# Lillthorin/YoloLite-Official-Repo

Hardware: AMD Instinct MI355X
Metric: images/sec (higher is better)
Workload: dtype f32

## Files before the change

yololite-official-repo_amd/_lib.py:

```python
from __future__ import annotations

import ctypes as C
import os
import sys
import warnings


def _default_hw_queues():
    if "GPU_MAX_HW_QUEUES" in os.environ or os.environ.get("YOLOLITE_NO_ENV_DEFAULTS"):
        return
    os.environ["GPU_MAX_HW_QUEUES"] = "8"
    t = sys.modules.get("torch")
    try:
        late = t is not None and t.cuda.is_initialized()
    except Exception:
        late = False
    if late:
        warnings.warn("yololite_amd: the HIP runtime was initialised before this package was imported, so "
                      "GPU_MAX_HW_QUEUES=8 cannot be applied; export it in the environment (multi-stream overlap "
                      "of the executor degrades by ~25 % next to RCCL streams otherwise)", RuntimeWarning)


_default_hw_queues()

_HERE = os.path.dirname(os.path.abspath(__file__))
LIB_PATH = os.environ.get("YOLOLITE_HIP_LIB") or os.path.join(_HERE, "libyololite_hip.so")

YL_ABI_VERSION = 5
YL_MAX_LEVELS = 8
YL_OK = 0
ACT = {"none": 0, "relu": 1, "relu6": 2, "silu": 3, "gelu": 4, "relu_lab": 5}
OP_STEM, OP_CONV, OP_DW, OP_STEMBLOCK, OP_SE = 0, 1, 2, 3, 4
OP_POOL, OP_COPY, OP_LN, OP_GRN, OP_NHWC4 = 5, 6, 7, 8, 9
POST_MAIN, POST_FALLBACK, POST_EVAL = 0, 1, 2
CENTER = {"v8": 0, "simple": 1}
WH = {"softplus": 0, "v8": 1, "exp": 2}
NMS_TORCHVISION, NMS_GREEDY = 0, 1

DEV_DW_TILE_OFF, DEV_PWS_OFF, DEV_S2C_OFF, DEV_DWC_ALL, DEV_DWT_OFF = 1, 2, 4, 8, 16
DEV_DWT_NOSPLIT = 1 << 10
DEV_WINO_V1 = 1 << 11
DEV_DWL_OFF = 1 << 14
DEV_DWL_ALL = 1 << 15
DEV_DPW_OFF = 1 << 16
DEV_K3W_OFF = 1 << 17
DEV_POISON = 1 << 18
DEV_WINO_SHAPE_SHIFT = 12

_fp = C.POINTER(C.c_float)
_ip = C.POINTER(C.c_int32)


class yl_layer(C.Structure):
    _fields_ = [(n, C.c_int32) for n in (
        "op", "in_slot", "out_slot", "res_slot", "up_slot", "head_level", "cin", "cout",
        "k", "stride", "pad_t", "pad_l", "act", "in_shift", "dw_k", "dw_stride", "dw_pad_t", "dw_pad_l", "dw_act")] + [
        ("w", _fp), ("b", _fp), ("dw_w", _fp), ("dw_b", _fp),
        ("c2", C.c_int32), ("act2", C.c_int32), ("c3", C.c_int32), ("act3", C.c_int32),
        ("w2", _fp), ("b2", _fp), ("w3", _fp), ("b3", _fp), ("scale_slot", C.c_int32), ("reserved0", C.c_int32),
        ("lab_scale", C.c_float), ("lab_bias", C.c_float), ("eps", C.c_float), ("out_ch_off", C.c_int32)]


class yl_model_desc(C.Structure):
    _fields_ = [("abi_version", C.c_int32), ("img_size", C.c_int32), ("in_channels", C.c_int32),
                ("num_classes", C.c_int32), ("num_masks", C.c_int32), ("proto_slot", C.c_int32),
                ("num_levels", C.c_int32),
                ("level_size", C.c_int32 * YL_MAX_LEVELS), ("level_anchors", C.c_int32 * YL_MAX_LEVELS),
                ("num_slots", C.c_int32), ("slot_h", _ip), ("slot_w", _ip), ("slot_c", _ip),
                ("num_layers", C.c_int32), ("layers", C.POINTER(yl_layer))]


class yl_post_cfg(C.Structure):
    _fields_ = [("mode", C.c_int32), ("conf_thr", C.c_float), ("iou_thr", C.c_float),
                ("per_class_cap", C.c_int32), ("topk", C.c_int32), ("max_out", C.c_int32),
                ("center_mode", C.c_int32), ("wh_mode", C.c_int32), ("backmap_dev", C.c_void_p),
                ("fallback_nms", C.c_int32)]


_vp = C.c_void_p
# ... 79 lines not shown
```

yololite-official-repo_amd/csrc/yl_api.hip:

```cpp
#include "yl_internal.h"

#include <dlfcn.h>
#include <limits.h>
#include <math.h>
#include <stdio.h>
#include <stddef.h>
#include <string.h>

#include <algorithm>
#include <memory>
#include <chrono>
#include <string>
#include <vector>

#define YL_DW_LDS_MAX (32 * 1024)

namespace {

struct DevLayer {
  yl_layer d;
  float* wp = nullptr;
  float* bias = nullptr;
  float* dw_w = nullptr;
  float* dw_b = nullptr;
// ... 40 lines not shown
  bool plan_reuse = false;
  int opt_reuse = 1;
  int opt_time_split = 0;
  hipEvent_t ev_t[3] = {nullptr, nullptr, nullptr};
  bool timing_valid = false;
  int opt_pre_norm = 0;
  float* level_buf[YL_MAX_LEVELS] = {nullptr};
  float4* ws_boxes = nullptr;
  float* ws_scores = nullptr;
  int* ws_cls = nullptr;
  int* ws_clsws = nullptr;
  int* ws_kept_list = nullptr;
  int* ws_done = nullptr;
  unsigned long long* ws_gkeys = nullptr;
  int gP = 0;
  float* ws_tmp_dets = nullptr;
  int* ws_tmp_idx = nullptr;
  int post_cap_batch = 0;
  int* ws_nms_clsws = nullptr;
  unsigned long long* ws_nms_gkeys = nullptr;
  int nms_gP = 0;
  int opt_graph = 0, opt_tile_m = 0, opt_streams = 2;
  int opt_nms_groups = 0;
  int opt_hybrid = 0;
  int small_lo = 0, small_hi = 0;
  int tiny_lo = 0, tiny_hi = 0;
  int opt_batch_levels = 1;
  int opt_winograd = 1;
  int wino_max_hw = 0;
  int opt_fuse_decode = 1;
  int opt_fuse_head = 1;
  int opt_split_k = 0;
  int opt_dev = 0;
  int opt_bf16 = 0;
  hipStream_t work[4] = {nullptr, nullptr, nullptr, nullptr};
  hipEvent_t ev_fork = nullptr, ev_join[4] = {nullptr, nullptr, nullptr, nullptr};
  int opt_lanes = 0;
  std::vector<unsigned char> lane;
  hipStream_t side[4] = {nullptr, nullptr, nullptr, nullptr};
  hipEvent_t ev_la[4] = {nullptr, nullptr, nullptr, nullptr}, ev_lb[4] = {nullptr, nullptr, nullptr, nullptr};
  struct GraphEntry {
    std::vector<hipGraphExec_t> execs;
    int n = 0;
    std::vector<unsigned char> key;
    unsigned long long stamp = 0;
  };
  std::vector<GraphEntry> graphs;
  unsigned long long graph_clock = 0;
  std::shared_ptr<int> weights_owner;
  std::string err;
};

namespace {

bool g_inited[64] = {false};

yl_status fail(yl_ctx* c, yl_status s, const std::string& msg) {
  if (c) c->err = msg;
  return s;
}

#define HIPCHK(ctx, expr)                                                                        \
  do {                                                                                           \
    hipError_t _e = (expr);                                                                      \
    if (_e != hipSuccess) {                                                                      \
      char _b[512];                                                                              \
// ... 116 lines not shown
    hipFree(c->arena[i]); c->arena[i] = nullptr; c->arena_capi[i] = 0;
    hipFree(c->se_scratch[i]); c->se_scratch[i] = nullptr;
  }
  for (auto& s : c->slots) { hipFree(s.pin); s.pin = nullptr; }
  for (int l = 0; l < YL_MAX_LEVELS; ++l) { hipFree(c->level_buf[l]); c->level_buf[l] = nullptr; }
  c->cap_batch = 0; c->plan_n = 0; c->arena_n = 0; c->arena_cap = 0; c->act_batch = 0;
}

int pow2ceil(int v) { int p = 64; while (p < v) p <<= 1; return p; }

size_t layer_group_end(const yl_ctx* c, size_t i, size_t lend) {
  auto same_shape = [&](size_t x, size_t y) {
    const yl_layer& a = c->layers[x].d; const yl_layer& e = c->layers[y].d;
    return a.op == YL_OP_CONV && e.op == YL_OP_CONV && a.cin == e.cin && a.cout == e.cout && a.k == e.k &&
           a.stride == e.stride && a.pad_t == e.pad_t && a.pad_l == e.pad_l && a.act == e.act &&
           !YL_ACT_POSTPASS(a.act) && a.in_shift == e.in_shift && a.dw_k == e.dw_k && a.dw_stride == e.dw_stride && a.dw_pad_t == e.dw_pad_t &&
           a.dw_pad_l == e.dw_pad_l && a.dw_act == e.dw_act && a.c2 == 0 && e.c2 == 0 && a.scale_slot < 0 && e.scale_slot < 0 && a.res_slot < 0 &&
           e.res_slot < 0 && a.up_slot < 0 && e.up_slot < 0 && (a.head_level >= 0) == (e.head_level >= 0) &&
           (a.cout + 15) / 16 <= 8;
  };
  size_t gend = i + 1;
  if (c->layers[i].d.op != YL_OP_CONV) return gend;
  while (gend < lend && gend - i < 4 && same_shape(i, gend)) {
    bool dep = false;
    for (size_t q = i; q < gend; ++q)
      if (c->layers[q].d.head_level < 0 && c->layers[q].d.out_slot == c->layers[gend].d.in_slot) dep = true;
    if (dep) break;
    ++gend;
  }
  return gend;
}

bool pair_fusable(const yl_ctx* c, size_t i, size_t lend, bool ignore_options);

void plan_slots(yl_ctx* c, bool reuse) {
  const size_t NL = c->layers.size(), NS = c->slots.size();
  std::vector<int> grp(NL, 0);
  int g = 0;
  for (size_t i = 0; i < NL; ++g) {
    size_t e = layer_group_end(c, i, NL);
    if (pair_fusable(c, e - 1, NL, true)) e = e + 1;
    for (size_t q = i; q < e; ++q) grp[q] = g;
    i = e;
  }
  const int INF = 1 << 30;
  std::vector<int> def(NS, INF), last(NS, -1);
  for (size_t i = 0; i < NL; ++i) {
    const yl_layer& d = c->layers[i].d;
    if (d.head_level < 0 && d.out_slot >= 0 && grp[i] < def[d.out_slot]) def[d.out_slot] = grp[i];
    const int ins[4] = {(d.op == YL_OP_STEM || d.op == YL_OP_STEMBLOCK || d.op == YL_OP_NHWC4) ? -1 : d.in_slot, d.res_slot, d.up_slot, d.scale_slot};
    for (int k = 0; k < 4; ++k)
      if (ins[k] >= 0 && grp[i] > last[ins[k]]) last[ins[k]] = grp[i];
  }
  for (size_t s = 0; s < NS; ++s) {
    Slot& t = c->slots[s];
    t.pinned = (int)s == c->proto_slot;
    bool f32 = c->opt_bf16 != 3 || t.pinned;
    for (size_t i = 0; i < NL && !f32; ++i) f32 = c->layers[i].d.op == YL_OP_SE && c->layers[i].d.out_slot == (int)s;
    t.sz = (size_t)t.h * t.w * t.c * (f32 ? sizeof(float) : sizeof(_Float16));
    if (last[s] < def[s]) last[s] = def[s] == INF ? -1 : def[s];
  }
  struct Iv { size_t off, sz; int last; };
  std::vector<Iv> live;
  size_t peak = 0;
  std::vector<size_t> order;
  for (size_t s = 0; s < NS; ++s) if (!c->slots[s].pinned && def[s] != INF) order.push_back(s);
  std::stable_sort(order.begin(), order.end(), [&](size_t a, size_t b) { return def[a] < def[b]; });
  size_t bump = 0;
  for (size_t s : order) {
    Slot& t = c->slots[s];
    const size_t need = (t.sz + 255) & ~(size_t)255;
    if (!reuse) { t.off = bump; bump += need; peak = bump; continue; }
    live.erase(std::remove_if(live.begin(), live.end(), [&](const Iv& v) { return v.last < def[s]; }), live.end());
    std::sort(live.begin(), live.end(), [](const Iv& a, const Iv& b) { return a.off < b.off; });
// ... 214 lines not shown
      return false;
    if (T.in_h != T.out_h || T.in_w != T.out_w || !yl_dpp_supported(t.cin, t.cout, o.cout, T.out_h, T.out_w)) return false;
    for (size_t r = 0; r < c->layers.size(); ++r) {
      if (r == gend + q) continue;
      const yl_layer& e = c->layers[r].d;
      const bool reads_in = e.op != YL_OP_STEM && e.op != YL_OP_STEMBLOCK && e.in_slot == t.out_slot;
      if (reads_in || e.res_slot == t.out_slot || e.up_slot == t.out_slot) return false;
    }
  }
  return true;
}

bool pair_fusable(const yl_ctx* c, size_t i, size_t lend, bool ignore_options) {
  if ((!ignore_options && (!c->opt_fuse_head || c->opt_bf16)) || i + 1 >= lend) return false;
  const DevLayer& T = c->layers[i];
  const yl_layer& t = T.d; const yl_layer& o = c->layers[i + 1].d;
  if (t.op != YL_OP_CONV || t.k != 1 || t.dw_k != 3 || t.dw_stride != 1 || t.c2 > 0 || t.c3 > 0 || t.head_level >= 0 ||
      t.res_slot >= 0 || t.up_slot >= 0 || t.in_shift || YL_SMOOTH(t.act) || YL_SMOOTH(t.dw_act) || t.out_slot < 0)
    return false;
  if (o.op != YL_OP_CONV || o.head_level >= 0 || o.k != 1 || o.dw_k > 0 || o.c2 > 0 || o.c3 > 0 || o.in_slot != t.out_slot ||
      o.cin != t.cout || YL_SMOOTH(o.act) || o.up_slot >= 0 || o.in_shift || o.res_slot == t.out_slot ||
      o.scale_slot >= 0 || t.scale_slot >= 0)
    return false;
  if (T.in_h != T.out_h || T.in_w != T.out_w || !yl_dpq_supported(t.cin, t.cout, o.cout, T.out_h, T.out_w)) return false;
  for (size_t r = 0; r < c->layers.size(); ++r) {
    if (r == i + 1) continue;
    const yl_layer& e = c->layers[r].d;
    const bool reads_in = e.op != YL_OP_STEM && e.op != YL_OP_STEMBLOCK && e.in_slot == t.out_slot;
    if (reads_in || e.res_slot == t.out_slot || e.up_slot == t.out_slot) return false;
  }
  return true;
}

hipError_t conv_multi(const yl_ctx* c, const YlConvP* ps, int n, hipStream_t st) {
  switch (c->opt_bf16) {
    case 1: return yl_launch_conv_multi_bf16(ps, n, c->opt_tile_m, st);
    case 2: return yl_launch_conv_multi_f16(ps, n, c->opt_tile_m, st);
    case 3: return yl_launch_conv_multi_f16s(ps, n, c->opt_tile_m, st);
    default: return yl_launch_conv_multi(ps, n, c->opt_tile_m, st);
  }
}

yl_status run_layers(yl_ctx* c, const float* x, int b0, int B, float* const* level_out, hipStream_t st,
                     hipEvent_t* evs , int chunk = 0,
                     const yl_post_cfg* fuse = nullptr ,
                     int lo = 0, int hi = -1 ) {
  if (evs) HIPCHK(c, hipEventRecord(evs[0], st));
  const bool lanes = !evs && c->opt_lanes && !c->lane.empty() && chunk >= 0 && chunk < 4;
  hipStream_t sd = nullptr;
  if (lanes) {
    if (!c->side[chunk]) HIPCHK(c, hipStreamCreateWithFlags(&c->side[chunk], hipStreamNonBlocking));
    if (!c->ev_la[chunk]) HIPCHK(c, hipEventCreateWithFlags(&c->ev_la[chunk], hipEventDisableTiming));
    if (!c->ev_lb[chunk]) HIPCHK(c, hipEventCreateWithFlags(&c->ev_lb[chunk], hipEventDisableTiming));
    sd = c->side[chunk];
  }
  std::vector<unsigned char> prod(c->slots.size(), 0);
  bool side_used = false;
  int pooled_slot = -1, pooled_P = 0;
  auto params = [&](size_t i, YlConvP& p) {
    layer_params(c, c->layers[i], b0, B, x, level_out, p);
    const yl_layer& d = c->layers[i].d;
    if (fuse && d.head_level >= 0) {
      const int l = d.head_level, S = c->level_S[l];
      const size_t o = (size_t)b0 * c->N;
      p.dec_boxes = c->ws_boxes + o; p.dec_scores = c->ws_scores + o; p.dec_cls = c->ws_cls + o;
      p.dec_N = c->N; p.dec_off = c->level_off[l] + c->layers[i].head_anchor * S * S; p.dec_C = c->C;
// ... 31 lines not shown
      const hipError_t e = yl_launch_conv_dpp(ps, (int)n, st);
      if (e == hipSuccess) { i = gend + n; continue; }
      if (e != hipErrorNotSupported) {
        char b[256];
        snprintf(b, sizeof(b), "layers %zu..%zu head launch failed: %s", i, gend + n - 1, hipGetErrorString(e));
        return fail(c, YL_ERR_HIP, b);
      }
    }
    if (!evs && !lanes && gend == i + 1 && d.op == YL_OP_CONV && d.dw_k == 3 && d.dw_stride == 1 && d.k == 1 && d.c2 == 0 &&
        d.c3 == 0 && c->opt_fuse_head && !c->opt_bf16 && d.head_level < 0 && d.res_slot < 0 && d.up_slot < 0 && !d.in_shift &&
        d.cout > 96 && !pair_fusable(c, i, lend, false) && c->layers[i].in_h == c->layers[i].out_h &&
        yl_dpq_supported(d.cin, d.cout, 0, c->layers[i].out_h, c->layers[i].out_w)) {
      YlConvP pt;
      params(i, pt);
      pt.w3p = nullptr;
      const hipError_t e = yl_launch_conv_dpq(pt, st);
      if (e == hipSuccess) { ++i; continue; }
      if (e != hipErrorNotSupported) {
        char b[256];
        snprintf(b, sizeof(b), "layer %zu launch failed: %s", i, hipGetErrorString(e));
        return fail(c, YL_ERR_HIP, b);
      }
    }
    if (!evs && !lanes && gend == i + 1 && d.op == YL_OP_CONV && d.dw_k == 3 && pair_fusable(c, i, lend, false)) {
      YlConvP pt, po;
      params(i, pt);
      params(i + 1, po);
      pt.w3p = po.wp; pt.b3 = po.bias; pt.C3 = po.N; pt.act3 = po.act; pt.res = po.res; pt.out = po.out;
      const hipError_t e = yl_launch_conv_dpq(pt, st);
      if (e == hipSuccess) { i += 2; continue; }
      if (e != hipErrorNotSupported) {
        char b[256];
        snprintf(b, sizeof(b), "layers %zu..%zu fused launch failed: %s", i, i + 1, hipGetErrorString(e));
        return fail(c, YL_ERR_HIP, b);
      }
    }
    if (fuse && !evs && !lanes && d.op == YL_OP_CONV && d.head_level >= 0 && c->layers[i].wp_det && c->opt_fuse_head) {
      bool all = true;
      for (size_t q = i; q < gend; ++q) all = all && c->layers[q].wp_det != nullptr;
      if (all) {
        YlConvP pd[4];
        const int nd = 5 + c->C;
        for (size_t q = i; q < gend; ++q) {
          YlConvP o;
          params(q, o);
          YlConvP& a = pd[q - i];
          a = o; a.wp = c->layers[q].wp_det; a.bias = c->layers[q].b_det; a.N = nd; a.NTtot = cdiv(nd, 16); a.dec_raw = 0;
          a.w3p = c->layers[q].wp_mc; a.b3 = c->layers[q].b_mc; a.C3 = c->NM;
          a.out = o.out + nd; a.ldo = c->E;
        }
        const int n = (int)(gend - i);
        const hipError_t e = conv_multi(c, pd, n, st);
        if (e != hipSuccess) {
          char b[256];
          snprintf(b, sizeof(b), "layers %zu..%zu split head launch failed: %s", i, gend - 1, hipGetErrorString(e));
          return fail(c, YL_ERR_HIP, b);
        }
        i = gend;
        continue;
      }
    }
    if (gend - i > 1) {
      YlConvP ps[4];
      for (size_t q = i; q < gend; ++q) params(q, ps[q - i]);
      const hipError_t e = conv_multi(c, ps, (int)(gend - i), st);
      if (e != hipSuccess) {
// ... 863 lines not shown
    const int nv = value ? 3 : (c->opt_bf16 == 3 ? 0 : c->opt_bf16);
    if ((nv == 3) != (c->opt_bf16 == 3)) free_act(c);
    c->opt_bf16 = nv; drop_graph(c); return YL_OK;
  }
  if (!strcmp(name, "nms_groups")) { c->opt_nms_groups = value < 0 ? 0 : (value > YL_NMS_GROUPS ? YL_NMS_GROUPS : value); drop_graph(c); return YL_OK; }
  if (!strcmp(name, "time_split")) {
    c->opt_time_split = value ? 1 : 0;
    for (int i = 0; i < 3 && value; ++i)
      if (!c->ev_t[i]) HIPCHK(c, hipEventCreate(&c->ev_t[i]));
    c->timing_valid = false;
    return YL_OK;
  }
  if (!strcmp(name, "pre_norm")) { c->opt_pre_norm = value ? 1 : 0; return YL_OK; }
  if (!strcmp(name, "reuse_slots")) { c->opt_reuse = value ? 1 : 0; drop_graph(c); return YL_OK; }
  if (!strcmp(name, "hybrid")) { c->opt_hybrid = value < 0 ? 0 : (value > 2 ? 2 : value); drop_graph(c); return YL_OK; }
  if (!strcmp(name, "batch_levels")) { c->opt_batch_levels = value ? 1 : 0; drop_graph(c); return YL_OK; }
  if (!strcmp(name, "fuse_decode")) { c->opt_fuse_decode = value ? 1 : 0; drop_graph(c); return YL_OK; }
  if (!strcmp(name, "fuse_head")) { c->opt_fuse_head = value ? 1 : 0; drop_graph(c); return YL_OK; }
  if (!strcmp(name, "winograd")) { c->opt_winograd = value < 0 ? 0 : (value > 2 ? 2 : value); drop_graph(c); return YL_OK; }
  if (!strcmp(name, "lanes")) { c->opt_lanes = value ? 1 : 0; drop_graph(c); return YL_OK; }
  if (!strcmp(name, "tile_m")) { c->opt_tile_m = value; drop_graph(c); return YL_OK; }
  if (!strcmp(name, "streams")) { c->opt_streams = value < 1 ? 1 : (value > 4 ? 4 : value); drop_graph(c); return YL_OK; }
  if (!strcmp(name, "split_k")) { c->opt_split_k = value ? 1 : 0; drop_graph(c); return YL_OK; }
  if (!strcmp(name, "dev_select")) { c->opt_dev = value & (int)YL_DEV_MASK; drop_graph(c); return YL_OK; }
  return fail(c, YL_ERR_INVALID, std::string("unknown option ") + name);
}

yl_status yl_get_option(const yl_ctx* c, const char* name, int32_t* value) {
  if (!c || !name || !value) return YL_ERR_INVALID;
  const struct { const char* n; int v; } tab[] = {
      {"graph", c->opt_graph}, {"mfma_bf16", c->opt_bf16 == 1}, {"mfma_f16", c->opt_bf16 == 2}, {"store_f16", c->opt_bf16 == 3}, {"nms_groups", c->opt_nms_groups}, {"time_split", c->opt_time_split},
      {"pre_norm", c->opt_pre_norm}, {"reuse_slots", c->opt_reuse}, {"hybrid", c->opt_hybrid}, {"batch_levels", c->opt_batch_levels},
      {"fuse_decode", c->opt_fuse_decode}, {"fuse_head", c->opt_fuse_head}, {"winograd", c->opt_winograd}, {"lanes", c->opt_lanes},
      {"tile_m", c->opt_tile_m}, {"streams", c->opt_streams}, {"dev_select", c->opt_dev}, {"split_k", c->opt_split_k}};
  for (const auto& t : tab)
    if (!strcmp(name, t.n)) { *value = t.v; return YL_OK; }
  return YL_ERR_INVALID;
}

int32_t yl_query_fused_block(int32_t c_in, int32_t c_mid, int32_t c_out, int32_t dw_k, int32_t dw_stride, int32_t out_h,
                             int32_t out_w) {
  if (c_in < 1 || c_mid < 1 || c_out < 1 || out_h < 1 || out_w < 1) return 0;
  if (yl_ir_supported(c_in, c_mid, c_out, dw_k, dw_stride, out_h, out_w)) return 1;
  if (dw_stride == 1 && !(out_h & 3) && !(out_w & 3) && yl_uib_supported(c_in, c_mid, c_out, dw_k)) return 2;
  return 0;
}

int32_t yl_query_dw_prologue(int32_t c_in, int32_t c_out, int32_t dw_k, int32_t dw_stride, int32_t out_h, int32_t out_w) {
  if (c_in < 1 || c_out < 1 || dw_k < 1 || dw_stride < 1 || out_h < 1 || out_w < 1) return 0;
  if (yl_dws_supported(c_in, c_out, dw_k, dw_stride, out_h, out_w)) return 2;
  if ((size_t)(dw_k * dw_k + 1) * c_in * sizeof(float) <= YL_DW_LDS_MAX) return 1;
  return 0;
}

static yl_status forward_impl(yl_ctx* c, const float* x, int B, float* const* level_out, hipStream_t st,
                              float* layer_ms, const yl_post_cfg* cfg, float* dets, int* counts, int* keep_idx = nullptr) {
  if (!c) return YL_ERR_INVALID;
  if (c->layers.empty()) return fail(c, YL_ERR_STATE, "context was created without layers");
  if (!x || B < 1) return fail(c, YL_ERR_INVALID, "bad input");
  HIPCHK(c, hipSetDevice(c->device));
  yl_status s = ensure_act(c, B, layer_ms ? 1 : chunks_for(c, B));
  if (s != YL_OK) return s;
  if (cfg && (s = ensure_post(c, B)) != YL_OK) return s;
  if ((s = poison_act(c, st)) != YL_OK) return s;
  Job j;
  j.x = x; j.B = B; j.cfg = cfg; j.dets = dets; j.counts = counts; j.keep_idx = keep_idx;
  for (int l = 0; l < c->L; ++l) j.outs[l] = (level_out && level_out[l]) ? level_out[l] : c->level_buf[l];
// ... 206 lines not shown
```

yololite-official-repo_amd/csrc/yl_convc.hip:

```cpp
#include "yl_lp.h"
#if defined(YL_BF16) && YL_BF16
#define yl_conv_dwc_kernel YL_LP_NAME(yl_conv_dwc_kernel)
#define yl_launch_conv_dwc YL_LP_NAME(yl_launch_conv_dwc)
#define yl_convc_init YL_LP_NAME(yl_convc_init)
#define yl_conv_pwt_kernel YL_LP_NAME(yl_conv_pwt_kernel)
#define yl_launch_conv_pwt YL_LP_NAME(yl_launch_conv_pwt)
#define yl_launch_conv_pwt_multi YL_LP_NAME(yl_launch_conv_pwt_multi)
#define yl_conv_dwt_kernel YL_LP_NAME(yl_conv_dwt_kernel)
#define yl_launch_conv_dwt YL_LP_NAME(yl_launch_conv_dwt)
#define yl_conv_dwk_kernel YL_LP_NAME(yl_conv_dwk_kernel)
#define yl_conv_dwl_kernel YL_LP_NAME(yl_conv_dwl_kernel)
#define yl_launch_conv_dwk YL_LP_NAME(yl_launch_conv_dwk)
#define yl_conv_dws_kernel YL_LP_NAME(yl_conv_dws_kernel)
#define yl_launch_conv_dws YL_LP_NAME(yl_launch_conv_dws)
#define yl_conv_wino_kernel YL_LP_NAME(yl_conv_wino_kernel)
#define yl_launch_conv_wino YL_LP_NAME(yl_launch_conv_wino)
#define yl_conv_kxk_kernel YL_LP_NAME(yl_conv_kxk_kernel)
#define yl_launch_conv_kxk YL_LP_NAME(yl_launch_conv_kxk)
#define yl_conv_pws_kernel YL_LP_NAME(yl_conv_pws_kernel)
#define yl_launch_conv_pws YL_LP_NAME(yl_launch_conv_pws)
#define yl_ir_kernel YL_LP_NAME(yl_ir_kernel)
#define yl_launch_conv_ir YL_LP_NAME(yl_launch_conv_ir)
#define yl_ir_supported YL_LP_NAME(yl_ir_supported)
#endif
// ... 447 lines not shown
  const YlConvP& p = ps[0];
  const int NT = p.NTtot;
  const bool dec = p.dec_boxes != nullptr;
  int ntw = dec ? (NT <= 4 ? NT : 6) : (NT <= 4 ? NT : (NT % 4 == 0 ? 4 : (NT % 3 == 0 ? 3 : 4)));
  const int nchunk = dec ? 1 : (NT + ntw - 1) / ntw;
  const bool two = Mtot >= 65536;
  if (dec) {
    switch (ntw) {
      case 1: return pwt_go<1, 1, true>(m, nchunk, st);
      case 2: return pwt_go<2, 1, true>(m, nchunk, st);
      case 3: return pwt_go<3, 1, true>(m, nchunk, st);
      case 4: return pwt_go<4, 1, true>(m, nchunk, st);
      default: return two ? pwt_go<6, 2, true>(m, nchunk, st) : pwt_go<6, 1, true>(m, nchunk, st);
    }
  }
  if (p.scale) {
    switch (ntw) {
      case 1: return pwt_go<1, 1, false, true>(m, nchunk, st);
      case 2: return pwt_go<2, 1, false, true>(m, nchunk, st);
      case 3: return pwt_go<3, 1, false, true>(m, nchunk, st);
      default: return pwt_go<4, 1, false, true>(m, nchunk, st);
    }
  }
  switch (ntw) {
    case 1: return two ? pwt_go<1, 2>(m, nchunk, st) : pwt_go<1, 1>(m, nchunk, st);
    case 2: return two ? pwt_go<2, 2>(m, nchunk, st) : pwt_go<2, 1>(m, nchunk, st);
    case 3: return two ? pwt_go<3, 2>(m, nchunk, st) : pwt_go<3, 1>(m, nchunk, st);
    default: return two ? pwt_go<4, 2>(m, nchunk, st) : pwt_go<4, 1>(m, nchunk, st);
  }
}

hipError_t yl_launch_conv_pwt(const YlConvP& p, hipStream_t st) { return yl_launch_conv_pwt_multi(&p, 1, st); }

template <int NT, int DK, int DS, int MT, bool WL, int SK = 1>
__global__ __launch_bounds__(256, MT == 2 ? 2 : 3) void yl_conv_dwt_kernel(YlConvMulti mp) {
  YL_SELECT_PROBLEM_C(mp)
  constexpr int HPY = 3 * DS + DK, HPX = (4 * MT - 1) * DS + DK;
  constexpr int PITCHF = ((HPX * 16 + 7) / 64) * 64 + 56;
  constexpr int HF4 = HPY * HPX * 4;
  constexpr int NSLOT = (HF4 + 63) / 64;
  extern __shared__ __attribute__((aligned(16))) float yl_clds[];
  const int tid = threadIdx.x, lane = tid & 63;
  const int wave = __builtin_amdgcn_readfirstlane(tid >> 6);
  const int kq = lane >> 4, pl = lane & 15;
  const int Cin = p.Cin, H = p.H, W = p.W, OH = p.OH, OW = p.OW, N = p.N, NTtot = p.NTtot, KB = p.KB;
  const yl_act_t* const xin = p.x;
  const __amdgpu_buffer_rsrc_t xrs = __builtin_amdgcn_make_buffer_rsrc(
      const_cast<yl_act_t*>(p.x), 0, (int)((long)p.B * H * W * Cin * (long)sizeof(yl_act_t)), 0x00020000);
  constexpr unsigned OOB = 0x80000000u;
  f32x4* wl = reinterpret_cast<f32x4*>(yl_clds);
  float* dwl = yl_clds + (WL ? (size_t)KB * NTtot * 256 : 0);
  float* halo = dwl + (((size_t)(DK * DK + 1) * Cin + 3) & ~(size_t)3) + wave * (HPY * PITCHF);
  f32x4* red = reinterpret_cast<f32x4*>(dwl + (((size_t)(DK * DK + 1) * Cin + 3) & ~(size_t)3) + 4 * (HPY * PITCHF));
  const f32x4* wg = reinterpret_cast<const f32x4*>(p.wp);
  const int twn = OW / (4 * MT), thn = OH >> 2;
  const int tiles_img = twn * thn;
  const int ntiles = p.B * tiles_img;
  int tile, tend, wstride;
  constexpr int WPT = SK > 1 ? 1 : 4;
  if ((gx & 7) == 0) {
    const int tpx = (ntiles + 7) >> 3;
    const int band0 = (bx & 7) * tpx;
    tend = (band0 + tpx) < ntiles ? (band0 + tpx) : ntiles;
    tile = band0 + (bx >> 3) * WPT + (SK > 1 ? 0 : wave);
    wstride = (gx >> 3) * WPT;
  } else {
    tile = bx * WPT + (SK > 1 ? 0 : wave); tend = ntiles; wstride = gx * WPT;
  }
// ... 141 lines not shown
            }
          }
        }
      }
#pragma unroll
      for (int mt = 0; mt < MT; ++mt) xq[mt] = yl_sel4(c < Cin, yl_actc(xq[mt], dw_act, dlo, dhi));
      if (WL) {
        const f32x4* wrow = wl + (size_t)kb * NTtot * 64 + lane;
#pragma unroll
        for (int nt = 0; nt < NT; ++nt) wq[nt] = wrow[(nt < NTtot ? nt : NTtot - 1) * 64];
      }
      yl_mma_step<NT, MT>(wq, xq, acc);
      if (more) {
        __builtin_amdgcn_fence(__ATOMIC_ACQ_REL, "wavefront");
        stage_store(stg);
      }
    }
    if (SK > 1) {
      f32x4* rb = red + (size_t)(sk_par & 1u) * (4 * NT * 64);
#pragma unroll
      for (int nt = 0; nt < NT; ++nt) rb[(wave * NT + nt) * 64 + lane] = acc[0][nt];
      __syncthreads();
      ++sk_par;
#pragma unroll
      for (int nt = 0; nt < NT; ++nt) {
        if ((nt & (SK - 1)) != wave) continue;
        f32x4 one[1][1];
        one[0][0] = ((rb[(0 * NT + nt) * 64 + lane] + rb[(1 * NT + nt) * 64 + lane]) + rb[(2 * NT + nt) * 64 + lane]) +
                    rb[(3 * NT + nt) * 64 + lane];
        const YlPix px1[1] = {px[0]};
        if (!pre_add && (p.res || p.up || YL_SMOOTH(p.act))) yl_epi_generic<1, 1>(p, one, px1, nt, kq);
        else yl_epi_fast<1, 1>(p, one, px1, nt, kq, lo, hi, true);
      }
    } else {
      if (!pre_add && (p.res || p.up || YL_SMOOTH(p.act))) yl_epi_generic<NT, MT>(p, acc, px, 0, kq);
      else yl_epi_fast<NT, MT>(p, acc, px, 0, kq, lo, hi, true);
    }
    txi += sdx;
    if (txi >= twn) { txi -= twn; ++tyi; }
    tyi += sdy;
    if (tyi >= thn) { tyi -= thn; ++tb; }
    tb += sdb;
  }
}

template <int NT, int DK, int DS, int MT, bool WL, int SK = 1>
static hipError_t dwt_go(YlConvMulti& m, hipStream_t st, bool attr_only) {
  if (attr_only)
    return hipFuncSetAttribute((const void*)yl_conv_dwt_kernel<NT, DK, DS, MT, WL, SK>, hipFuncAttributeMaxDynamicSharedMemorySize, 96 * 1024);
  constexpr int HPY = 3 * DS + DK, HPX = (4 * MT - 1) * DS + DK;
  constexpr int PITCHF = ((HPX * 16 + 7) / 64) * 64 + 56;
  const YlConvP& p = m.p[0];
  const size_t lds = ((WL ? (size_t)p.KB * p.NTtot * 256 : 0) + (((size_t)(DK * DK + 1) * p.Cin + 3) & ~(size_t)3) +
                      (size_t)4 * HPY * PITCHF + (SK > 1 ? (size_t)2 * 4 * NT * 256 : 0)) * 4;
  if (lds > 96 * 1024) return hipErrorNotSupported;
  const int res = yl_resident_blocks_n(yl_conv_dwt_kernel<NT, DK, DS, MT, WL, SK>, 256, lds);
  long tiles[4], total = 0;
  for (int k = 0; k < m.n; ++k) {
    tiles[k] = (long)m.p[k].B * (m.p[k].OH >> 2) * (m.p[k].OW / (4 * MT)) * (SK > 1 ? 4 : 1);
    total += tiles[k];
  }
  int at = 0;
  for (int k = 0; k < m.n; ++k) {
    long g = ((long)res * tiles[k] / total + 7) & ~7L;
    const long cap = ((tiles[k] + 3) / 4 + 7) & ~7L;
    if (g > cap) g = cap;
    if (g < 8) g = 8;
    m.p[k].blk0 = at;
    m.p[k].nblk = (int)g;
    at += (int)g;
  }
  if (m.n == 1) m.p[0].nblk = 0;
  hipLaunchKernelGGL((yl_conv_dwt_kernel<NT, DK, DS, MT, WL, SK>), dim3((unsigned)at), dim3(256), lds, st, m);
  return hipGetLastError();
}

// ... 44 lines not shown
  }
  return wl ? dwt_dk<NT, 1, true>(m, st, false) : dwt_dk<NT, 1, false>(m, st, false);
}

static hipError_t dwt_any(YlConvMulti& m, int NT, hipStream_t st, bool two, bool wl, bool attr_only) {
  hipError_t e = hipSuccess;
  if (attr_only || NT == 1) e = dwt_nt<1>(m, st, two, wl, attr_only);
  if (attr_only ? e == hipSuccess : NT == 2) e = dwt_nt<2>(m, st, two, wl, attr_only);
  if (attr_only ? e == hipSuccess : NT == 3) e = dwt_nt<3>(m, st, two, wl, attr_only);
  if (attr_only ? e == hipSuccess : NT == 4) e = dwt_nt<4>(m, st, two, wl, attr_only);
  if (attr_only ? e == hipSuccess : NT == 6) e = dwt_nt<6>(m, st, two, wl, attr_only);
  return e;
}

hipError_t yl_launch_conv_dwt(YlConvMulti& m, hipStream_t st) {
  const YlConvP& p = m.p[0];
  if (p.dw_k == 0 || (p.N & 3) || p.NTtot > 6 || p.dec_boxes || p.C1 > 0) return hipErrorNotSupported;
  if (p.dev & YL_DEV_DWT_OFF) return hipErrorNotSupported;
  bool two = false, wl = p.KB * p.NTtot <= 36;
  for (int k = 0; k < m.n; ++k) {
    if ((m.p[k].OH & 3) || (m.p[k].OW & 3)) return hipErrorNotSupported;
    if ((size_t)m.p[k].B * m.p[k].H * m.p[k].W * m.p[k].Cin * sizeof(yl_act_t) >= ((size_t)1 << 31)) return hipErrorNotSupported;
    if (m.p[k].OW & 7) two = false;
  }
  const int nts[5] = {1, 2, 3, 4, 6};
  int NT = 6;
  for (int i = 0; i < 5; ++i) if (nts[i] >= p.NTtot) { NT = nts[i]; break; }
  if (m.n == 1 && NT == 4 && !wl && p.KB >= 8 && p.OH * p.OW <= 400 && !(p.dev & YL_DEV_DWT_NOSPLIT)) {
    const hipError_t e = dwt_splitk(m, st, false);
    if (e != hipErrorNotSupported) return e;
  }
  return dwt_any(m, NT, st, two, wl, false);
}

template <int NT, int MT, int NW>
__global__ __launch_bounds__(NW * 64, NW == 4 ? 3 : 4) void yl_conv_kxk_kernel(YlConvP p) {
  extern __shared__ __attribute__((aligned(16))) float yl_clds[];
  const int tid = threadIdx.x, lane = tid & 63;
  const int wave = __builtin_amdgcn_readfirstlane(tid >> 6);
  const int kq = lane >> 4, pl = lane & 15;
  const int TK = p.TK, KB = p.KB, K = p.k, NTtot = p.NTtot;
  const int Cin = p.Cin, H = p.H, W = p.W, stride = p.stride, pad_t = p.pad_t, pad_l = p.pad_l, sh = p.in_shift;
  const int ohw = p.OH * p.OW, OW = p.OW, M = p.M;
  const yl_act_t* const xin = p.x;
  const long zdelta = p.zeros - p.x;
  f32x4* wl = reinterpret_cast<f32x4*>(yl_clds);
  const f32x4* wg = reinterpret_cast<const f32x4*>(p.wp);
  const int NC = 3 * KB;
  const int G = NTtot / NT;
  const int bx = blockIdx.x, gx = gridDim.x;
  const int per = gx >> 3, slot = bx >> 3;
  const int tpx = (p.ntiles + 7) >> 3;
  const int band0 = (bx & 7) * tpx;
  const int band1 = (band0 + tpx) < p.ntiles ? (band0 + tpx) : p.ntiles;
  const int bt = band1 > band0 ? band1 - band0 : 0;
  const int nitems = bt * G;
  const int nmine = slot < nitems ? (nitems - 1 - slot) / per + 1 : 0;
  const long total_chunks = (long)nmine * NC;

  auto load_chunk = [&](int g, int kb, int cc, int buf) {
    for (int i = wave; i < 3 * NT; i += NW) {
      const int j = i / NT, nt = i - j * NT;
      f32x4* dst = wl + ((size_t)buf * 3 * NT + i) * 64;
      yl_glds16(wg + ((size_t)((cc * 3 + j) * KB + kb) * NTtot + g * NT + nt) * 64 + lane, dst);
    }
  };
// ... 1855 lines not shown
  return attr_only ? hipSuccess : hipErrorInvalidValue;
}

int kbmax_of(int ntw) { return ntw == 1 ? 18 : ntw == 2 ? 9 : ntw == 3 ? 6 : 4; }

}

hipError_t yl_convc_init() {
  YlConvMulti m = {};
  YlConvP q = {};
  hipError_t e = kxk_go<7, 1, 4>(q, 1, nullptr, true);
  if (e == hipSuccess) e = kxk_go<7, 2, 4>(q, 1, nullptr, true);
  if (e == hipSuccess) e = kxk_go<7, 1, 8>(q, 1, nullptr, true);
  if (e == hipSuccess) e = kxk_go<4, 1, 8>(q, 1, nullptr, true);
  if (e == hipSuccess) e = kxk_go<4, 2, 4>(q, 1, nullptr, true);
  if (e == hipSuccess) e = yl_ir_init();
  if (e == hipSuccess) e = pws_nw<6>(q, nullptr, false, true);
  if (e == hipSuccess) e = pws_nw<7>(q, nullptr, false, true);
  if (e == hipSuccess) e = pws_nw<8>(q, nullptr, false, true);
  if (e == hipSuccess) e = pws_nw<9>(q, nullptr, false, true);
  if (e == hipSuccess) e = pws_nw<11>(q, nullptr, false, true);
  if (e == hipSuccess) e = pws_nw<13>(q, nullptr, false, true);
  if (e == hipSuccess) e = dwt_any(m, 0, nullptr, false, false, true);
  if (e == hipSuccess) e = dwt_splitk(m, nullptr, true);
  if (e == hipSuccess) e = wino_go(q, nullptr, true);
  if (e == hipSuccess) e = yl_wino2_init();
  if (e == hipSuccess) e = dwk_go<7, 1, 4>(q, nullptr, true);
  if (e == hipSuccess) e = dwk_go<7, 3, 4>(q, nullptr, true);
  if (e == hipSuccess) e = dwk_go<8, 1, 4>(q, nullptr, true);
  if (e == hipSuccess) e = dwk_go<8, 2, 4>(q, nullptr, true);
  if (e == hipSuccess) e = dwl_go<16>(q, nullptr, true);
  if (e == hipSuccess) e = dwl_go<21>(q, nullptr, true);
  if (e == hipSuccess) e = yl_dws_init();
  if (e != hipSuccess) return e;
  return dwc_any(m, 0, 0, 0, 0, 0, nullptr, true, nullptr);
}

hipError_t yl_launch_conv_dwc(YlConvMulti& m, hipStream_t st) {
  const YlConvP& p = m.p[0];
  const int ntw = (p.NTtot + 3) / 4;
  if (ntw < 1 || ntw > 5 || p.KB > kbmax_of(ntw) || (p.N & 3)) return hipErrorNotSupported;
  const bool all = (p.dev & YL_DEV_DWC_ALL) != 0;
  if (!all && (p.KB < 12 || p.dw_stride != 1)) return hipErrorNotSupported;
  if (!((p.dw_k == 3 || p.dw_k == 5) && (p.dw_stride == 1 || p.dw_stride == 2))) return hipErrorNotSupported;
  const int HP = 3 * p.dw_stride + p.dw_k;
  const int NG = (p.KB + 3) / 4;
  const int PITCH = p.dw_stride == 1 ? HP * 32 + ((HP * 128) % 256 == 128 ? 0 : 32) : HP * 32 + 16;
  const size_t lds = ((size_t)2 * p.KB * 256 + (((size_t)(p.dw_k * p.dw_k + 1) * p.Cin + 3) & ~(size_t)3) +
                      (size_t)(NG < 4 ? NG : 4) * HP * PITCH) * 4;
  if (lds > YL_DWC_LDS_MAX) return hipErrorNotSupported;
  long tiles[4], total = 0;
  for (int k = 0; k < m.n; ++k) {
    if ((m.p[k].OH & 3) || (m.p[k].OW & 3) || (size_t)m.p[k].B * m.p[k].H * m.p[k].W * m.p[k].Cin * 4 >= ((size_t)1 << 31))
      return hipErrorNotSupported;
    tiles[k] = (long)m.p[k].B * (m.p[k].OH >> 2) * (m.p[k].OW >> 2);
    total += tiles[k];
  }
  int res = 0;
  hipError_t e = dwc_any(m, ntw, p.dw_k, p.dw_stride, 0, lds, st, false, &res);
  if (e != hipSuccess) return e;
  long gx = (total + 7) & ~7L;
  if (gx > res) gx = res & ~7L;
  if (gx < 8) gx = 8;
  if (m.n == 1) { m.p[0].blk0 = 0; m.p[0].nblk = 0; }
  else {
    int at = 0;
// ... 12 lines not shown
```

yololite-official-repo_amd/csrc/yl_internal.h:

```cpp
#pragma once
#include <hip/hip_runtime.h>
#include <stdint.h>
#include "../../include/yololite_hip.h"

#define YL_SMOOTH(a) ((a) >= YL_ACT_SILU)
#define YL_ACT_POSTPASS(a) ((a) >= YL_ACT_GELU)

#define YL_NUM_CU 256
#define YL_LDS_KEYS_MAX 16384

struct YlLevels {
  const float* ptr[YL_MAX_LEVELS];
  int S[YL_MAX_LEVELS];
  int A[YL_MAX_LEVELS];
  int off[YL_MAX_LEVELS + 1];
  float stride[YL_MAX_LEVELS];
  int L, N, E, C;
  float hi;
};

struct YlDecodeP {
  int mode;
  int center_mode, wh_mode;
  float4* boxes;
// ... 70 lines not shown
  int* dec_cls;
  int dec_N;
  int dec_off;
  int dec_C;
  int dec_mode, dec_center, dec_wh;
  int dec_raw;
  float dec_stride, dec_hi;
  int blk0, nblk;
  const float* wino;
  const float* scale;
  unsigned dev;
  float* pool;
  int pool_wpi;
  int ldo;
  int out_f32;
};

#define YL_DEV_DW_TILE_OFF (1u << 0)
#define YL_DEV_PWS_OFF (1u << 1)
#define YL_DEV_S2C_OFF (1u << 2)
#define YL_DEV_DWC_ALL (1u << 3)
#define YL_DEV_DWT_OFF (1u << 4)
#define YL_DEV_DWK(d) (((d) >> 5) & 3u)
#define YL_DEV_KXK_NW(d) (((d) >> 7) & 3u)
#define YL_DEV_KXK_MT2 (1u << 9)
#define YL_DEV_DWT_NOSPLIT (1u << 10)
#define YL_DEV_WINO_V1 (1u << 11)
#define YL_DEV_WINO_SHAPE(d) (((d) >> 12) & 3u)
#define YL_DEV_DWL_OFF (1u << 14)
#define YL_DEV_DWL_ALL (1u << 15)
#define YL_DEV_DPW_OFF (1u << 16)
#define YL_DEV_K3W_OFF (1u << 17)
#define YL_DEV_POISON (1u << 18)
#define YL_DEV_MASK 0x3ffffffu
static_assert(YL_DEV_MASK <= 0x7fffffffu, "dev_select is stored in an int (and an int field of the graph key)");
static_assert(((YL_DEV_DW_TILE_OFF | YL_DEV_PWS_OFF | YL_DEV_S2C_OFF | YL_DEV_DWC_ALL | YL_DEV_DWT_OFF | (3u << 5) | (3u << 7) |
                YL_DEV_KXK_MT2 | YL_DEV_DWT_NOSPLIT | YL_DEV_WINO_V1 | (3u << 12) | YL_DEV_DWL_OFF | YL_DEV_DWL_ALL | YL_DEV_DPW_OFF |
                YL_DEV_K3W_OFF | YL_DEV_POISON) & ~YL_DEV_MASK) == 0, "a YL_DEV_* bit lies outside the dev_select mask");

struct YlSeP {
  const float* x;
  float* partial;
  const float* w1;
  const float* b1;
  const float* w2;
  const float* b2;
  float* gate;
  int B, HW, C, RD, P, act;
};
hipError_t yl_launch_se(const YlSeP& p, bool pooled, hipStream_t st);
int yl_se_parts(int HW, int C);
int yl_dw_pool_wpi(int k, int stride, int cin, int n, int oh, int ow);

struct YlOpP {
  const float* x;
  float* out;
  const float* w;
  const float* b;
  float* partial;
  int B, H, W, C, OH, OW;
  int k, stride, pad_t, pad_l;
  int ldo, ch_off;
  int P;
  float eps;
  const float* res;
  int act;
  float lab_s, lab_b;
};
#define YL_OP_ACTPASS 100
hipError_t yl_launch_op(int op, const YlOpP& p, hipStream_t st);
int yl_grn_parts(int HW);
// ... 20 lines not shown

hipError_t yl_launch_stem(const YlConvP& p, hipStream_t st);
hipError_t yl_launch_conv(const YlConvP& p, int tile_hint, hipStream_t st);
hipError_t yl_launch_conv_multi(const YlConvP* ps, int n, int tile_hint, hipStream_t st);
hipError_t yl_launch_dw(const YlConvP& p, hipStream_t st);
hipError_t yl_launch_stemblock(const YlConvP& p, hipStream_t st);
hipError_t yl_launch_stemdw(const YlConvP& p, hipStream_t st);
hipError_t yl_stemblock_init();
hipError_t yl_launch_conv_dpp(const YlConvP* ps, int n, hipStream_t st);
bool yl_dpp_supported(int cin, int cout, int c3, int oh, int ow);
hipError_t yl_dpp_init();
hipError_t yl_launch_conv_s2c(const YlConvP& p, hipStream_t st);
hipError_t yl_launch_conv_dpq(const YlConvP& p, hipStream_t st);
hipError_t yl_launch_conv_k3w(const YlConvP& p, hipStream_t st);
bool yl_dpq_supported(int cin, int cmid, int cout, int oh, int ow);
bool yl_stemblock_supported(int c1, int c2, int c3);
hipError_t yl_conv_init();
bool yl_uib_supported(int c1, int cmid, int n, int dk);
hipError_t yl_launch_conv_dwc(YlConvMulti& m, hipStream_t st);
hipError_t yl_launch_conv_dwc_bf16(YlConvMulti& m, hipStream_t st);
hipError_t yl_launch_conv_pwt(const YlConvP& p, hipStream_t st);
hipError_t yl_launch_conv_pwt_bf16(const YlConvP& p, hipStream_t st);
hipError_t yl_launch_conv_pwt_multi(const YlConvP* ps, int n, hipStream_t st);
hipError_t yl_launch_conv_pwt_multi_bf16(const YlConvP* ps, int n, hipStream_t st);
hipError_t yl_launch_conv_ir(const YlConvP& p, hipStream_t st);
hipError_t yl_launch_conv_ir_bf16(const YlConvP& p, hipStream_t st);
bool yl_ir_supported(int c1, int cmid, int n, int dk, int ds, int oh, int ow);
hipError_t yl_launch_conv_pws(const YlConvP& p, hipStream_t st);
hipError_t yl_launch_conv_pws_bf16(const YlConvP& p, hipStream_t st);
hipError_t yl_launch_conv_kxk(const YlConvP& p, hipStream_t st);
hipError_t yl_launch_conv_kxk_bf16(const YlConvP& p, hipStream_t st);
hipError_t yl_launch_conv_dwt(YlConvMulti& m, hipStream_t st);
hipError_t yl_launch_conv_dwt_bf16(YlConvMulti& m, hipStream_t st);
hipError_t yl_launch_conv_dwk(const YlConvP& p, hipStream_t st);
hipError_t yl_launch_conv_dwk_bf16(const YlConvP& p, hipStream_t st);
hipError_t yl_launch_conv_dws(const YlConvP& p, hipStream_t st);
hipError_t yl_launch_conv_dws_bf16(const YlConvP& p, hipStream_t st);
hipError_t yl_launch_conv_dws_f16(const YlConvP& p, hipStream_t st);
bool yl_dws_supported(int cin, int n, int dk, int ds, int oh, int ow);
hipError_t yl_launch_conv_wino(const YlConvP& p, hipStream_t st);
hipError_t yl_launch_conv_wino_bf16(const YlConvP& p, hipStream_t st);
hipError_t yl_convc_init();
hipError_t yl_convc_init_bf16();
hipError_t yl_launch_conv_bf16(const YlConvP& p, int tile_hint, hipStream_t st);
hipError_t yl_launch_conv_multi_bf16(const YlConvP* ps, int n, int tile_hint, hipStream_t st);
hipError_t yl_conv_init_bf16();
hipError_t yl_launch_stemblock_bf16(const YlConvP& p, hipStream_t st);
hipError_t yl_launch_stemdw_bf16(const YlConvP& p, hipStream_t st);
hipError_t yl_stemblock_init_bf16();
hipError_t yl_launch_conv_f16(const YlConvP& p, int tile_hint, hipStream_t st);
hipError_t yl_launch_conv_multi_f16(const YlConvP* ps, int n, int tile_hint, hipStream_t st);
hipError_t yl_conv_init_f16();
hipError_t yl_convc_init_f16();
hipError_t yl_launch_stemblock_f16(const YlConvP& p, hipStream_t st);
hipError_t yl_launch_stemdw_f16(const YlConvP& p, hipStream_t st);
hipError_t yl_stemblock_init_f16();
hipError_t yl_launch_conv_f16s(const YlConvP& p, int tile_hint, hipStream_t st);
hipError_t yl_launch_conv_multi_f16s(const YlConvP* ps, int n, int tile_hint, hipStream_t st);
hipError_t yl_launch_stem_f16s(const YlConvP& p, hipStream_t st);
hipError_t yl_launch_dw_f16s(const YlConvP& p, hipStream_t st);
hipError_t yl_conv_init_f16s();
hipError_t yl_convc_init_f16s();
hipError_t yl_launch_stemblock_f16s(const YlConvP& p, hipStream_t st);
hipError_t yl_launch_stemdw_f16s(const YlConvP& p, hipStream_t st);
hipError_t yl_stemblock_init_f16s();
```

Before: 47460.

## Chain depthwise+pointwise conv with following 1x1 expand conv in one kernel

```diff
diff --git a/yololite-official-repo_amd/_lib.py b/yololite-official-repo_amd/_lib.py
--- a/yololite-official-repo_amd/_lib.py
+++ b/yololite-official-repo_amd/_lib.py
@@ -45,6 +45,7 @@
 DEV_DPW_OFF = 1 << 16
 DEV_K3W_OFF = 1 << 17
 DEV_POISON = 1 << 18
+DEV_CHAIN_OFF = 1 << 19
 DEV_WINO_SHAPE_SHIFT = 12
 
 _fp = C.POINTER(C.c_float)
diff --git a/yololite-official-repo_amd/csrc/yl_api.hip b/yololite-official-repo_amd/csrc/yl_api.hip
--- a/yololite-official-repo_amd/csrc/yl_api.hip
+++ b/yololite-official-repo_amd/csrc/yl_api.hip
@@ -96,6 +96,7 @@
   int opt_fuse_head = 1;
   int opt_split_k = 0;
   int opt_dev = 0;
+  int chain_launches = 0;
   int opt_bf16 = 0;
   hipStream_t work[4] = {nullptr, nullptr, nullptr, nullptr};
   hipEvent_t ev_fork = nullptr, ev_join[4] = {nullptr, nullptr, nullptr, nullptr};
@@ -278,6 +279,7 @@
 }
 
 bool pair_fusable(const yl_ctx* c, size_t i, size_t lend, bool ignore_options);
+bool chain_fusable(const yl_ctx* c, size_t i, size_t lend, bool ignore_options);
 
 void plan_slots(yl_ctx* c, bool reuse) {
   const size_t NL = c->layers.size(), NS = c->slots.size();
@@ -285,7 +287,7 @@
   int g = 0;
   for (size_t i = 0; i < NL; ++g) {
     size_t e = layer_group_end(c, i, NL);
-    if (pair_fusable(c, e - 1, NL, true)) e = e + 1;
+    if (pair_fusable(c, e - 1, NL, true) || chain_fusable(c, e - 1, NL, true)) e = e + 1;
     for (size_t q = i; q < e; ++q) grp[q] = g;
     i = e;
   }
@@ -566,6 +568,25 @@
   return true;
 }
 
+bool chain_fusable(const yl_ctx* c, size_t i, size_t lend, bool ignore_options) {
+  if (!ignore_options && (c->opt_bf16 || c->opt_split_k || c->opt_tile_m || (c->opt_dev & (YL_DEV_CHAIN_OFF | YL_DEV_DWT_OFF))))
+    return false;
+  if (i + 1 >= lend) return false;
+  const DevLayer& T = c->layers[i];
+  const DevLayer& O = c->layers[i + 1];
+  const yl_layer& t = T.d; const yl_layer& o = O.d;
+  if (t.op != YL_OP_CONV || t.k != 1 || t.stride != 1 || t.dw_k <= 0 || t.dw_stride != 1 || t.c2 > 0 || t.c3 > 0 ||
+      t.head_level >= 0 || t.up_slot >= 0 || t.scale_slot >= 0 || t.in_shift || YL_SMOOTH(t.act) || t.out_slot < 0 ||
+      (t.res_slot >= 0 && t.act != YL_ACT_NONE))
+    return false;
+  if (o.op != YL_OP_CONV || o.head_level >= 0 || o.k != 1 || o.stride != 1 || o.dw_k > 0 || o.c2 > 0 || o.c3 > 0 ||
+      o.in_slot != t.out_slot || o.cin != t.cout || YL_SMOOTH(o.act) || o.res_slot >= 0 || o.up_slot >= 0 ||
+      o.scale_slot >= 0 || o.in_shift || o.out_slot < 0)
+    return false;
+  return T.in_h == T.out_h && T.in_w == T.out_w && O.in_h == T.out_h && O.in_w == T.out_w && O.out_h == T.out_h &&
+         O.out_w == T.out_w && yl_dwx_supported(t.cin, t.cout, t.dw_k, t.dw_stride, o.cout, T.out_h, T.out_w);
+}
+
 hipError_t conv_multi(const yl_ctx* c, const YlConvP* ps, int n, hipStream_t st) {
   switch (c->opt_bf16) {
     case 1: return yl_launch_conv_multi_bf16(ps, n, c->opt_tile_m, st);
@@ -663,6 +684,19 @@
       if (e != hipErrorNotSupported) {
         char b[256];
         snprintf(b, sizeof(b), "layers %zu..%zu fused launch failed: %s", i, i + 1, hipGetErrorString(e));
+        return fail(c, YL_ERR_HIP, b);
+      }
+    }
+    if (!evs && !lanes && gend == i + 1 && d.op == YL_OP_CONV && d.dw_k > 0 && chain_fusable(c, i, lend, false)) {
+      YlConvP pt, po;
+      params(i, pt);
+      params(i + 1, po);
+      pt.w3p = po.wp; pt.b3 = po.bias; pt.C3 = po.N; pt.act3 = po.act;
+      const hipError_t e = yl_launch_conv_dwx(pt, po.out, st);
+      if (e == hipSuccess) { ++c->chain_launches; i += 2; continue; }
+      if (e != hipErrorNotSupported) {
+        char b[256];
+        snprintf(b, sizeof(b), "layers %zu..%zu chained launch failed: %s", i, i + 1, hipGetErrorString(e));
         return fail(c, YL_ERR_HIP, b);
       }
     }
@@ -1592,7 +1626,8 @@
       {"graph", c->opt_graph}, {"mfma_bf16", c->opt_bf16 == 1}, {"mfma_f16", c->opt_bf16 == 2}, {"store_f16", c->opt_bf16 == 3}, {"nms_groups", c->opt_nms_groups}, {"time_split", c->opt_time_split},
       {"pre_norm", c->opt_pre_norm}, {"reuse_slots", c->opt_reuse}, {"hybrid", c->opt_hybrid}, {"batch_levels", c->opt_batch_levels},
       {"fuse_decode", c->opt_fuse_decode}, {"fuse_head", c->opt_fuse_head}, {"winograd", c->opt_winograd}, {"lanes", c->opt_lanes},
-      {"tile_m", c->opt_tile_m}, {"streams", c->opt_streams}, {"dev_select", c->opt_dev}, {"split_k", c->opt_split_k}};
+      {"tile_m", c->opt_tile_m}, {"streams", c->opt_streams}, {"dev_select", c->opt_dev}, {"split_k", c->opt_split_k},
+      {"chain_launches", c->chain_launches}};
   for (const auto& t : tab)
     if (!strcmp(name, t.n)) { *value = t.v; return YL_OK; }
   return YL_ERR_INVALID;
diff --git a/yololite-official-repo_amd/csrc/yl_convc.hip b/yololite-official-repo_amd/csrc/yl_convc.hip
--- a/yololite-official-repo_amd/csrc/yl_convc.hip
+++ b/yololite-official-repo_amd/csrc/yl_convc.hip
@@ -503,8 +503,57 @@
 
 hipError_t yl_launch_conv_pwt(const YlConvP& p, hipStream_t st) { return yl_launch_conv_pwt_multi(&p, 1, st); }
 
-template <int NT, int DK, int DS, int MT, bool WL, int SK = 1>
-__global__ __launch_bounds__(256, MT == 2 ? 2 : 3) void yl_conv_dwt_kernel(YlConvMulti mp) {
+template <int NT, int NX>
+__device__ __forceinline__ void yl_dwx_tail(const YlConvP& p, const f32x4 (&acc)[NT], size_t lin, int kq, int lane, float lo,
+                                            float hi, yl_act_t* const out3) {
+#if !YL_BF16
+  constexpr int CX = 2, NC = NX / CX;
+  static_assert(NX % CX == 0, "chained n-tiles come in chunks of CX");
+  const __amdgpu_buffer_rsrc_t wrs = __builtin_amdgcn_make_buffer_rsrc(const_cast<float*>(p.w3p), 0, NT * NX * 1024, 0x00020000);
+  const __amdgpu_buffer_rsrc_t ors =
+      __builtin_amdgcn_make_buffer_rsrc(out3, 0, (int)((long)p.B * p.OH * p.OW * NX * 64), 0x00020000);
+  f32x4 w[2][NT][CX];
+  auto wload = [&](int c, f32x4 (&d)[NT][CX]) {
+#pragma unroll
+    for (int kb = 0; kb < NT; ++kb)
+#pragma unroll
+      for (int j = 0; j < CX; ++j)
+        d[kb][j] = __builtin_bit_cast(f32x4, __builtin_amdgcn_raw_buffer_load_b128(wrs, lane * 16 + (c * CX + j) * 1024, kb * NX * 1024, 0));
+  };
+  wload(0, w[0]);
+  f32x4 hq[NT][1];
+  const size_t orow = lin * (size_t)p.N;
+#pragma unroll
+  for (int nt = 0; nt < NT; ++nt) {
+    const int n = nt * 16 + 4 * kq;
+    hq[nt][0] = yl_clamp4(acc[nt] + yl_ld4(p.bias + n), lo, hi);
+    yl_out4(p, orow + n, hq[nt][0]);
+  }
+  const float lo3 = (p.act3 == YL_ACT_RELU || p.act3 == YL_ACT_RELU6) ? 0.0f : -INFINITY;
+  const float hi3 = (p.act3 == YL_ACT_RELU6) ? 6.0f : INFINITY;
+  const int ob = (int)lin * (NX * 64) + kq * 16;
+#pragma unroll
+  for (int c = 0; c < NC; ++c) {
+    if (c + 1 < NC) wload(c + 1, w[(c + 1) & 1]);
+    f32x4 a[1][CX];
+#pragma unroll
+    for (int j = 0; j < CX; ++j) a[0][j] = (f32x4){0.f, 0.f, 0.f, 0.f};
+#pragma unroll
+    for (int kb = 0; kb < NT; ++kb) yl_mma_step<CX, 1>(w[c & 1][kb], hq[kb], a);
+#pragma unroll
+    for (int j = 0; j < CX; ++j) {
+      const f32x4 v = yl_clamp4(a[0][j] + yl_ld4(p.b3 + (c * CX + j) * 16 + 4 * kq), lo3, hi3);
+      __builtin_amdgcn_raw_buffer_store_b128(__builtin_bit_cast(__attribute__((ext_vector_type(4))) unsigned, v), ors,
+                                             ob + (c * CX + j) * 64, 0, 0);
+    }
+  }
+#else
+  (void)p; (void)acc; (void)lin; (void)kq; (void)lane; (void)lo; (void)hi; (void)out3;
+#endif
+}
+
+template <int NT, int DK, int DS, int MT, bool WL, int SK, int NX>
+__device__ __forceinline__ void yl_dwt_body(const YlConvMulti& mp, yl_act_t* const out3) {
   YL_SELECT_PROBLEM_C(mp)
   constexpr int HPY = 3 * DS + DK, HPX = (4 * MT - 1) * DS + DK;
   constexpr int PITCHF = ((HPX * 16 + 7) / 64) * 64 + 56;
@@ -712,6 +761,8 @@
         if (!pre_add && (p.res || p.up || YL_SMOOTH(p.act))) yl_epi_generic<1, 1>(p, one, px1, nt, kq);
         else yl_epi_fast<1, 1>(p, one, px1, nt, kq, lo, hi, true);
       }
+    } else if constexpr (NX > 0) {
+      yl_dwx_tail<NT, NX>(p, acc[0], px[0].lin, kq, lane, lo, hi, out3);
     } else {
       if (!pre_add && (p.res || p.up || YL_SMOOTH(p.act))) yl_epi_generic<NT, MT>(p, acc, px, 0, kq);
       else yl_epi_fast<NT, MT>(p, acc, px, 0, kq, lo, hi, true);
@@ -722,6 +773,11 @@
     if (tyi >= thn) { tyi -= thn; ++tb; }
     tb += sdb;
   }
+}
+
+template <int NT, int DK, int DS, int MT, bool WL, int SK = 1>
+__global__ __launch_bounds__(256, MT == 2 ? 2 : 3) void yl_conv_dwt_kernel(YlConvMulti mp) {
+  yl_dwt_body<NT, DK, DS, MT, WL, SK, 0>(mp, nullptr);
 }
 
 template <int NT, int DK, int DS, int MT, bool WL, int SK = 1>
@@ -832,6 +888,67 @@
   }
   return dwt_any(m, NT, st, two, wl, false);
 }
+
+#if !YL_BF16
+template <int DK, int NX>
+__global__ __launch_bounds__(256, 3) void yl_conv_dwx_kernel(YlConvMulti mp, float* out3) {
+  yl_dwt_body<4, DK, 1, 1, false, 1, NX>(mp, out3);
+}
+
+template <int DK, int NX>
+static hipError_t dwx_go(YlConvMulti& m, float* out3, hipStream_t st, bool attr_only) {
+  if (attr_only)
+    return hipFuncSetAttribute((const void*)yl_conv_dwx_kernel<DK, NX>, hipFuncAttributeMaxDynamicSharedMemorySize, 96 * 1024);
+  constexpr int HPY = 3 + DK, HPX = 3 + DK;
+  constexpr int PITCHF = ((HPX * 16 + 7) / 64) * 64 + 56;
+  YlConvP& p = m.p[0];
+  const size_t lds = ((((size_t)(DK * DK + 1) * p.Cin + 3) & ~(size_t)3) + (size_t)4 * HPY * PITCHF) * 4;
+  const int res = yl_resident_blocks_n(yl_conv_dwx_kernel<DK, NX>, 256, lds);
+  const long tiles = (long)p.B * (p.OH >> 2) * (p.OW >> 2);
+  long g = ((long)res + 7) & ~7L;
+  const long cap = ((tiles + 3) / 4 + 7) & ~7L;
+  if (g > cap) g = cap;
+  if (g < 8) g = 8;
+  p.blk0 = 0; p.nblk = 0;
+  hipLaunchKernelGGL((yl_conv_dwx_kernel<DK, NX>), dim3((unsigned)g), dim3(256), lds, st, m, out3);
+  return hipGetLastError();
+}
+
+bool yl_dwx_supported(int cin, int cout, int dw_k, int dw_stride, int cout1, int oh, int ow) {
+  return (cin == 192 || cin == 256) && cout == 64 && (dw_k == 3 || dw_k == 5) && dw_stride == 1 && (cout1 == 192 || cout1 == 256) &&
+         (oh & 3) == 0 && (ow & 3) == 0;
+}
+
+hipError_t yl_launch_conv_dwx(const YlConvP& pd, float* out3, hipStream_t st) {
+  const YlConvP& p = pd;
+  if (p.k != 1 || p.stride != 1 || p.C1 > 0 || p.up || p.scale || p.dec_boxes || p.ldo || p.in_shift || !p.w3p || !out3 ||
+      YL_SMOOTH(p.act) || YL_SMOOTH(p.act3) || (p.res && p.act != YL_ACT_NONE) || p.H != p.OH || p.W != p.OW ||
+      !yl_dwx_supported(p.Cin, p.N, p.dw_k, p.dw_stride, p.C3, p.OH, p.OW))
+    return hipErrorNotSupported;
+  if ((p.dev & (YL_DEV_DWT_OFF | YL_DEV_CHAIN_OFF)) || !(p.dev & YL_DEV_DWT_NOSPLIT) || p.KB * p.NTtot <= 36) return hipErrorNotSupported;
+  if ((size_t)p.B * p.H * p.W * p.Cin * sizeof(float) >= ((size_t)1 << 31) ||
+      (size_t)p.B * p.OH * p.OW * p.C3 * sizeof(float) >= ((size_t)1 << 31))
+    return hipErrorNotSupported;
+  YlConvMulti m = {};
+  m.n = 1;
+  m.p[0] = p;
+  const int nx = p.C3 / 16;
+  if (p.dw_k == 5 && nx == 16) return dwx_go<5, 16>(m, out3, st, false);
+  if (p.dw_k == 5 && nx == 12) return dwx_go<5, 12>(m, out3, st, false);
+  if (p.dw_k == 3 && nx == 16) return dwx_go<3, 16>(m, out3, st, false);
+  if (p.dw_k == 3 && nx == 12) return dwx_go<3, 12>(m, out3, st, false);
+  return hipErrorNotSupported;
+}
+
+static hipError_t yl_dwx_init() {
+  YlConvMulti m = {};
+  hipError_t e = dwx_go<5, 16>(m, nullptr, nullptr, true);
+  if (e == hipSuccess) e = dwx_go<5, 12>(m, nullptr, nullptr, true);
+  if (e == hipSuccess) e = dwx_go<3, 16>(m, nullptr, nullptr, true);
+  if (e == hipSuccess) e = dwx_go<3, 12>(m, nullptr, nullptr, true);
+  return e;
+}
+#endif
 
 template <int NT, int MT, int NW>
 __global__ __launch_bounds__(NW * 64, NW == 4 ? 3 : 4) void yl_conv_kxk_kernel(YlConvP p) {
@@ -2753,6 +2870,9 @@
   if (e == hipSuccess) e = dwl_go<16>(q, nullptr, true);
   if (e == hipSuccess) e = dwl_go<21>(q, nullptr, true);
   if (e == hipSuccess) e = yl_dws_init();
+#if !YL_BF16
+  if (e == hipSuccess) e = yl_dwx_init();
+#endif
   if (e != hipSuccess) return e;
   return dwc_any(m, 0, 0, 0, 0, 0, nullptr, true, nullptr);
 }
diff --git a/yololite-official-repo_amd/csrc/yl_internal.h b/yololite-official-repo_amd/csrc/yl_internal.h
--- a/yololite-official-repo_amd/csrc/yl_internal.h
+++ b/yololite-official-repo_amd/csrc/yl_internal.h
@@ -126,11 +126,12 @@
 #define YL_DEV_DPW_OFF (1u << 16)
 #define YL_DEV_K3W_OFF (1u << 17)
 #define YL_DEV_POISON (1u << 18)
+#define YL_DEV_CHAIN_OFF (1u << 19)
 #define YL_DEV_MASK 0x3ffffffu
 static_assert(YL_DEV_MASK <= 0x7fffffffu, "dev_select is stored in an int (and an int field of the graph key)");
 static_assert(((YL_DEV_DW_TILE_OFF | YL_DEV_PWS_OFF | YL_DEV_S2C_OFF | YL_DEV_DWC_ALL | YL_DEV_DWT_OFF | (3u << 5) | (3u << 7) |
                 YL_DEV_KXK_MT2 | YL_DEV_DWT_NOSPLIT | YL_DEV_WINO_V1 | (3u << 12) | YL_DEV_DWL_OFF | YL_DEV_DWL_ALL | YL_DEV_DPW_OFF |
-                YL_DEV_K3W_OFF | YL_DEV_POISON) & ~YL_DEV_MASK) == 0, "a YL_DEV_* bit lies outside the dev_select mask");
+                YL_DEV_K3W_OFF | YL_DEV_POISON | YL_DEV_CHAIN_OFF) & ~YL_DEV_MASK) == 0, "a YL_DEV_* bit lies outside the dev_select mask");
 
 struct YlSeP {
   const float* x;
@@ -217,6 +218,8 @@
 hipError_t yl_launch_conv_kxk_bf16(const YlConvP& p, hipStream_t st);
 hipError_t yl_launch_conv_dwt(YlConvMulti& m, hipStream_t st);
 hipError_t yl_launch_conv_dwt_bf16(YlConvMulti& m, hipStream_t st);
+hipError_t yl_launch_conv_dwx(const YlConvP& pd, float* out3, hipStream_t st);
+bool yl_dwx_supported(int cin, int cout, int dw_k, int dw_stride, int cout1, int oh, int ow);
 hipError_t yl_launch_conv_dwk(const YlConvP& p, hipStream_t st);
 hipError_t yl_launch_conv_dwk_bf16(const YlConvP& p, hipStream_t st);
 hipError_t yl_launch_conv_dws(const YlConvP& p, hipStream_t st);
```

New measurement: 48360, median of 6. 1.02x the previous value.
